# Aikku93/ulc-codec

Measured on AMD Instinct MI355X. Metric: encode+decode Msamples/s at BlockSize=2048 stereo (channel-samples through encode+decode, VBR -50, 32 blocks per stream per call), higher is better.
Workload: dtype f32; 1 GPU; vbr50 (configs[1] encode, configs[2] decode): Batch=4096 independent 44.1 kHz stereo streams/GPU x 32 blocks, BlockSize=2048, VBR -50; step = encode then decode; config=vbr50, mode=both, streams_per_gpu=4096, block_size=2048, channels=2, parallelism=batch split over 1 GPU(s), no collective on the data path

## Files before the change

ulc-codec_amd/csrc/ulcx_enc.hip:

```cpp
#include "ulcx_enc_dev.h"

static size_t ulcx_enc_xf_lds_bytes(int BS, int C) {
    if (BS > 8192) return (size_t)BS * 4;
    int ps = ulcx_xf_pad_shift(BS, C);
    size_t z = (size_t)4 * (BS + (BS >> ps)) * 4;
    size_t full = z + (size_t)BS * 2 + 32 + (C > 2 ? (size_t)BS * 2 : 0);
    return full <= ULCX_LDS_LIMIT ? full : z + (size_t)BS * 2 + 32;
}

static size_t ulcx_enc_xfa_lds_bytes(int BS, int C) {
    if (BS > 8192) return (size_t)BS * 4;
    int ps = ulcx_xf_pad_shift(BS, C);
    return (size_t)2 * (BS + (BS >> ps)) * 4 + (size_t)BS * 2 + 32;
}

#define CK(x) do { hipError_t e_ = (x); if (e_ != hipSuccess) { ulcx_set_error("%s: %s", #x, hipGetErrorString(e_)); return ULCX_ERR_HIP; } } while (0)
#define TRY(x) do { int rc_ = (x); if (rc_) return rc_; } while (0)

typedef void (*RangeKernel)(UlcxEncCtx, int, int);
typedef void (*PassKernel)(UlcxEncCtx, int);
typedef void (*CallKernel)(UlcxEncCtx);

static RangeKernel wc_energy_fn(const UlcxEncCtx &c) { return c.pcm16 ? k_wc_energy<int16_t> : k_wc_energy<float>; }
static RangeKernel wc_ef_fn(const UlcxEncCtx &c) { return c.pcm16 ? k_wc_ef<EF_NW, int16_t> : k_wc_ef<EF_NW, float>; }
// ... 25 lines not shown
    return pass == 1 ? select_fn_pass<1>(c, pair, rates) : pass == 2 ? select_fn_pass<2>(c, pair, rates) : select_fn_pass<0>(c, pair, rates);
}

static int allow_lds(const void *fn, size_t lds) {
    if (lds > 48 * 1024) CK(hipFuncSetAttribute(fn, hipFuncAttributeMaxDynamicSharedMemorySize, (int)lds));
    return ULCX_OK;
}

static void launch_wc_energy(const UlcxEncCtx &c, unsigned grid, hipStream_t st, int k0, int k1) {
    hipLaunchKernelGGL(wc_energy_fn(c), dim3(grid), dim3(WG), 0, st, c, k0, k1);
}

static void launch_wc_ef(const UlcxEncCtx &c, hipStream_t st, int k0, int k1) {
    static_assert(EF_LDS_BYTES <= 48 * 1024, "k_wc_ef: raise the dynamic LDS limit with hipFuncSetAttribute");
    hipLaunchKernelGGL(wc_ef_fn(c), dim3((c.B + EF_SPW - 1) / EF_SPW), dim3(EF_NW * 64), EF_LDS_BYTES, st, c, k0, k1);
}

static void launch_state_update(const UlcxEncCtx &c, hipStream_t st) {
    hipLaunchKernelGGL(state_update_fn(c), dim3(c.B), dim3(WG), 0, st, c);
}

const char *const ulcx_enc_stage_names[ULCX_ENC_STAGES_REPORTED] = {
    "k_wc_energy", "k_wc_forward", "k_wc_backward", "k_wc_integrate", "k_wc_decide",
    "k_xf", "k_cplx", "k_pbark", "k_mask",
    "k_select", "k_nbark", "(k_nline: gone)", "k_heapsel", "k_nsums", "k_tails", "k_encode_wave", "k_encode_units", "k_pack", "cbr_probe_passes", "k_state_update", "wc_pipeline_exposed",
};

struct StageMarks { hipEvent_t *ev; int stage; };
#define MARK(mk, s) do { if ((mk).ev) CK(hipEventRecord((mk).ev[(mk).stage++], s)); } while (0)

// ... 55 lines not shown
        hipLaunchKernelGGL(k_wc_integrate, dim3((c.B + 63) / 64), dim3(64), 0, side3, c, k0, k1);
        hipLaunchKernelGGL(k_wc_decide, dim3((c.B * kc + 63) / 64), dim3(64), 0, side3, c, k0, k1);
        CK(hipEventRecord(sy.wcDecided[w], side3));
        while (jx < nCh && cut[jx + 1] <= k1) {
            CK(hipStreamWaitEvent(st, sy.wcDecided[w], 0));
            if (mk.ev) CK(hipEventRecord(sy.xfTiming[2 * jx], st));
            if (!(ULCX_DBG(c) & 0x2000))
            transform(cut[jx], cut[jx + 1]);
            if (mk.ev) CK(hipEventRecord(sy.xfTiming[2 * jx + 1], st));
            CK(hipEventRecord(sy.xfChunkDone[jx], st));
            jx++;
        }
    }
    aux.nXf = nCh;
    MARK(mk, st);
    for (int j = 0; j < nCh; j++) {
        CK(hipStreamWaitEvent(side, sy.xfChunkDone[j], 0));
        const int kc2 = cut[j + 1] - cut[j];
        if (what == ULCX_FRONT_ENCODE) hipLaunchKernelGGL(k_cplx, dim3((c.B * kc2 + 63) / 64), dim3(64), 0, side, c, cut[j], cut[j + 1]);
        else hipLaunchKernelGGL(k_cplxa, dim3((c.B * kc2 + 63) / 64), dim3(64), 0, side, c, cut[j], cut[j + 1]);
    }
    CK(hipEventRecord(sy.cplxChunksDone, side));
    return ULCX_OK;
}

struct EncPlan {
    int NB, N, nUnits;
    bool aside;
    int probes;
    size_t barkLds;
    bool selWave, selPair;
    size_t selLds;
    int ldsEntries, fbGrid; size_t heapLds;
    WaveCaps capS, capM, capF;
    bool haveFull, haveMid;
// ... 27 lines not shown
    p.haveMid = p.capM.k < p.capF.k;
    p.nsSlots = aux.nsSlots;
    return p;
}

static void launch_noise(const UlcxEncCtx &c, const EncPlan &p, hipStream_t s2) {
    if (c.barkRing) {
        hipLaunchKernelGGL(k_bark_uniform<true>, dim3((p.NB * c.C + 63) / 64), dim3(256), p.barkLds, s2, c);
        hipLaunchKernelGGL(k_bark_levels<true>, dim3((unsigned)(((size_t)p.NB * c.C * 32 + WG - 1) / WG)), dim3(WG), 0, s2, c);
    }
    hipLaunchKernelGGL(k_nbark, dim3((p.nUnits + 63) / 64), dim3(64), 0, s2, c, c.barkRing ? 1 : 0);
}

static int launch_psy(const UlcxEncCtx &c, const EncPlan &p, UlcxEncSync &sy, hipStream_t st, StageMarks &mk, bool cplxChunked) {
    if (c.barkRing) { TRY(allow_lds((const void *)k_bark_uniform<true>, p.barkLds)); TRY(allow_lds((const void *)k_bark_uniform<false>, p.barkLds)); }
    if (p.aside) {
        CK(hipEventRecord(sy.noiseFork, st));
        CK(hipStreamWaitEvent(sy.side3, sy.noiseFork, 0));
        if (cplxChunked) CK(hipStreamWaitEvent(sy.side3, sy.cplxChunksDone, 0));
        else hipLaunchKernelGGL(k_cplx, dim3((p.NB + 63) / 64), dim3(64), 0, sy.side3, c, 0, c.K);
        CK(hipEventRecord(sy.cplxDone, sy.side3));
        MARK(mk, st);
        launch_state_update(c, sy.side3);
        CK(hipEventRecord(sy.stateDone, sy.side3));
        CK(hipStreamWaitEvent(sy.side2, sy.noiseFork, 0));
        launch_noise(c, p, sy.side2);
        CK(hipEventRecord(sy.noiseDone, sy.side2));
    } else { hipLaunchKernelGGL(k_cplx, dim3((p.NB + 63) / 64), dim3(64), 0, st, c, 0, c.K);                MARK(mk, st); }
    const bool uniP = c.barkRing != 0;
    if (uniP) {
        hipLaunchKernelGGL(k_bark_uniform<false>, dim3((p.NB + 63) / 64), dim3(256), p.barkLds, st, c);
        hipLaunchKernelGGL(k_bark_levels<false>, dim3((unsigned)(((size_t)p.NB * 32 + WG - 1) / WG)), dim3(WG), 0, st, c);
    }
    hipLaunchKernelGGL(k_pbark, dim3((p.NB * 4 + 63) / 64), dim3(64), 0, st, c, uniP ? 1 : 0);            MARK(mk, st);
    MARK(mk, st);
    if (p.aside) CK(hipStreamWaitEvent(st, sy.cplxDone, 0));
    return ULCX_OK;
}

static int launch_select_wave(const UlcxEncCtx &c, const EncPlan &p, hipStream_t st, bool rates, int pass, int fin) {
    const PassKernel fn = select_fn(c, p.selPair, rates, pass);
    TRY(allow_lds((const void *)fn, p.selLds));
    if (p.selPair) hipLaunchKernelGGL(fn, dim3(p.NB), dim3(128), p.selLds, st, c, fin);
// ... 144 lines not shown
    CK(hipGetLastError());
    return ULCX_OK;
}

int ulcx_enc_launch(const UlcxEncCtx &c, hipStream_t st, hipEvent_t *ev, const UlcxEncAux &aux) {
    return ulcx_enc_launch_ladder(&c, 1, st, ev, aux);
}

int ulcx_analyse_launch(const UlcxEncCtx &c, hipStream_t st, hipEvent_t *ev, const UlcxEncAux &aux, int useKxf) {
    const int what = !c.cplxOut ? ULCX_FRONT_WC_ONLY : useKxf ? ULCX_FRONT_ANALYSE_KXF : ULCX_FRONT_ANALYSE;
    if (what == ULCX_FRONT_ANALYSE_KXF && c.barkRing) CK(hipMemsetAsync(c.decCount, 0, sizeof(int), st));
    StageMarks mk = { ev, 0 };
    MARK(mk, st);
    TRY(launch_front(c, st, mk, aux, what));
    if (aux.wcPipe > 1) CK(hipStreamWaitEvent(st, aux.sync.cplxChunksDone, 0));
    else hipLaunchKernelGGL(k_cplxa, dim3((c.B * c.K + 63) / 64), dim3(64), 0, st, c, 0, c.K);
    MARK(mk, st);
    while (mk.ev && mk.stage < ULCX_ENC_STAGES) MARK(mk, st);
    launch_state_update(c, st);
    MARK(mk, st);
    CK(hipGetLastError());
    return ULCX_OK;
}
```

ulc-codec_amd/csrc/ulcx_enc_dev.h:

```cpp
#pragma once
#include <utility>
#include "ulcx_internal.h"

#include <type_traits>

#include "ulcx_libm.h"

#define WG 256

#define FFT_PACKED

#include "ulcx_fft.h"

__device__ __forceinline__ float fastlog(float x) {
    uint32_t b = __float_as_uint(x);
    int e = (int)(b >> 23) - 127;
    float m = __uint_as_float((127u << 23) | (b & 0x7FFFFFu));
    return -1.7417939f + (2.8212026f + (-1.4699568f + (0.44717955f - 0.056570851f * m) * m) * m) * m + 0.6931471806f * e;
}

__device__ __forceinline__ int quant_u(float v) {
    return (v >= 0.5f) ? (int)(0.5f + sqrtf(v - 0.25f)) : 0;
}

// ... 206 lines not shown
#define BK_PPR (BK_TL / 4)

#define BK_PIECES (64 * BK_PPR)

#define BK_NPC ((BK_PIECES + 191) / 192)

#ifndef BK_AHEAD

#define BK_AHEAD 4

#endif

#define BK_RS (2 * BK_TL + 4)

#define BK_TILE_FLOATS (64 * BK_RS)

__device__ __forceinline__ bool probes_over(const UlcxEncCtx &c, int finalPass) { return !finalPass && c.fbMode != 2 && *c.cbrLive <= 0; }

__device__ __forceinline__ bool skip_block(const UlcxEncCtx &c, int blk, int finalPass) {
    if (!finalPass && c.cbrDone[blk]) return true;
    if (c.fbMode == 1) return c.isFb[blk] != 0;
    return false;
}

__device__ __forceinline__ int fb_count(const UlcxEncCtx &c) {
    int n = *c.fbCount; if (n > c.fbHi) n = c.fbHi;
    n -= c.fbLo; return n > 0 ? n : 0;
}

#define ULCX_DPP_STEPS(OP) \
// ... 208 lines not shown
```

ulc-codec_amd/csrc/ulcx_enc_xf.hip:

```cpp
#include "ulcx_enc_dev.h"

__device__ __forceinline__ int first_overlap(int wc, int BS) {
    unsigned p = ulcx_pattern(wc);
    int ov = BS >> (p & 7);
    if (p & 8) ov >>= (wc & 7);
    return ov;
}

__device__ __forceinline__ float win_apply(float x, int i, int S, int aL, int ovL, int aR, int ov,
                                           const float *__restrict__ rise, const float *__restrict__ fall) {
    if (i < S) return (i < aL) ? 0.0f : (i < aL + ovL) ? x * rise[i - aL] : x;
    int n = i - S;
    return (n < aR) ? x : (n < aR + ov) ? x * fall[n - aR] : 0.0f;
}

template <typename IN, int BSC, bool AN = false>
__device__ __forceinline__ int xf_fast(const UlcxEncCtx &c, float *lds, int s, int k, int blk, int tid) {
    constexpr int BS = BSC, S = BSC, M = BSC / 2, PS = 4, Mp = FFT_PADDEDS(M, PS);
    constexpr int LGM = BSC == 4096 ? 11 : 10;
    static_assert(BSC == 2048 || BSC == 4096, "sizes with a compile-time transform");
    static_assert(WG == 256 && (M / 2) % (2 * WG) == 0, "whole fold / epilogue trips per thread");
    float2 *z = (float2 *)lds;
    float2 *twl = (float2 *)(lds + (AN ? 2 : 4) * FFT_PADDEDS(BS, PS));
    float2 *zc0 = z, *zs0 = z + Mp, *zc1 = z + (AN ? 1 : 2) * Mp, *zs1 = z + 3 * Mp;
    const float2 *pre = c.T.pre[0];
    const float *rise = c.T.winRise + S, *fall = c.T.winFall + S;
    const IN *pcmS = pcm_base<IN>(c) + (size_t)s * c.K * BS * 2;
    const IN *frameLo = pcmS + (ptrdiff_t)(k - 2) * BS * 2, *frameHi = frameLo;
    if constexpr (std::is_same<IN, float>::value) {
        const float *histS = c.hist + (size_t)s * 2 * BS * 2;
        if (k < 2) frameLo = histS + (size_t)k * BS * 2;
        if (k < 1) frameHi = histS;
// ... 28 lines not shown
                const float vl = la - lb, wl = lb + la;
                const float v1 = hsel ? vl : vr, v2 = hsel ? vr : vl;
                const float w1 = hsel ? wl : wr, w2 = hsel ? wr : wl;
                float2 *zc = q ? zc1 : zc0, *zs = q ? zs1 : zs0;
                zc[FFT_PADS(n, PS)] = cmulc(make_float2(v1, v2), P);
                if constexpr (!AN) zs[FFT_PADS(n, PS)] = cmulc(make_float2(w2, w1), P);
            }
        }
    }
    __syncthreads();
    if constexpr (AN) { if (tid < 128) fft_wave_dif_ct<M, PS>(z + __builtin_amdgcn_readfirstlane(tid >> 6) * Mp, twl, tid & 63); }
    else fft_wave_dif_ct<M, PS>(z + __builtin_amdgcn_readfirstlane(tid >> 6) * Mp, twl, tid & 63);
    __syncthreads();
    float *coefO = c.coef + (size_t)blk * (2 * BS);
    constexpr float norm = 2.0f / S;
    int nnz = 0;
    if constexpr (AN) {
#pragma unroll
        for (int e0 = 0; e0 < M / 2; e0 += 2 * WG) {
            const int kA = e0 + 2 * tid, kB = e0 + 2 * tid + 1;
            const int kk2[2] = { kA, kB };
            float re[2][2][4];
#pragma unroll
            for (int u = 0; u < 2; u++) {
                const int k1 = kk2[u], k2 = M - 1 - k1;
                const int r1 = (int)(__brev((unsigned)k1) >> (32 - LGM)), r2 = (int)(__brev((unsigned)k2) >> (32 - LGM));
                const float2 P1 = pre[k1], P2 = pre[k2];
                const fft_v2f Pv1 = { P1.x, P1.y }, Pv2 = { P2.x, P2.y };
#pragma unroll
                for (int q = 0; q < 2; q++) {
                    const float2 *zc = q ? zc1 : zc0;
// ... 2 lines not shown
                    const float mdct[4] = { yc1.x, yc2.y, yc2.x, yc1.y };
#pragma unroll
                    for (int p = 0; p < 2; p++) {
                        const int slot = p ? (1 - u) : u;
                        re[q][p][2 * slot] = mdct[2*p] * norm; re[q][p][2 * slot + 1] = mdct[2*p+1] * norm;
                    }
                }
            }
            const int j1 = kA, j2 = M - 1 - kB;
#pragma unroll
            for (int q = 0; q < 2; q++) {
                stnt((float4 *)(coefO + q * BS + 2 * j1), make_float4(re[q][0][0], re[q][0][1], re[q][0][2], re[q][0][3]));
                stnt((float4 *)(coefO + q * BS + 2 * j2), make_float4(re[q][1][0], re[q][1][1], re[q][1][2], re[q][1][3]));
            }
        }
        return 0;
    }
#pragma unroll
    for (int e0 = 0; e0 < M / 2; e0 += 2 * WG) {
        const int kA = e0 + 2 * tid, kB = e0 + 2 * tid + 1;
        const int kk2[2] = { kA, kB };
        float re[2][2][4];
        float ns[2][2][2];
        float am[2][2] = { { 0.0f, 0.0f }, { 0.0f, 0.0f } };
#pragma unroll
        for (int u = 0; u < 2; u++) {
            const int k1 = kk2[u], k2 = M - 1 - k1;
            const int r1 = (int)(__brev((unsigned)k1) >> (32 - LGM)), r2 = (int)(__brev((unsigned)k2) >> (32 - LGM));
            const float2 P1 = pre[k1], P2 = pre[k2];
            const fft_v2f Pv1 = { P1.x, P1.y }, Pv2 = { P2.x, P2.y };
#pragma unroll
            for (int q = 0; q < 2; q++) {
                const float2 *zc = q ? zc1 : zc0, *zs = q ? zs1 : zs0;
                auto cm = [](float2 d, fft_v2f w) { const fft_v2f dv = { d.x, d.y }; const fft_v2f r = fft_cmulc_post_pk(dv, w); return make_float2(r.x, r.y); };
                const float2 yc1 = cm(zc[FFT_PADS(r1, PS)], Pv1), yc2 = cm(zc[FFT_PADS(r2, PS)], Pv2);
                const float2 ys1 = cm(zs[FFT_PADS(r1, PS)], Pv1), ys2 = cm(zs[FFT_PADS(r2, PS)], Pv2);
                const float mdct[4] = { yc1.x, yc2.y, yc2.x, yc1.y };
                const float mdst[4] = { ys1.x, ys2.y, ys2.x, ys1.y };
#pragma unroll
                for (int p = 0; p < 2; p++) {
                    const float re0 = mdct[2*p] * norm,   im0 = mdst[2*p] * norm;
                    const float re1 = mdct[2*p+1] * norm, im1 = mdst[2*p+1] * norm;
                    const float re0s = re0 * re0, im0s = im0 * im0, re1s = re1 * re1, im1s = im1 * im1;
                    const float a0 = re0s + im0s, a1 = re1s + im1s;
                    nnz += (fabsf(re0) < 0.5f * ULCX_COEF_EPS) ? 0 : 1;
                    nnz += (fabsf(re1) < 0.5f * ULCX_COEF_EPS) ? 0 : 1;
                    const int slot = p ? (1 - u) : u;
                    re[q][p][2 * slot] = re0; re[q][p][2 * slot + 1] = re1;
                    ns[q][p][slot] = a0 + a1;
                    am[p][slot] += a0; am[p][slot] += a1;
                }
            }
        }
        const int j1 = kA, j2 = M - 1 - kB;
#pragma unroll
        for (int q = 0; q < 2; q++) {
            stnt((float4 *)(coefO + q * BS + 2 * j1), make_float4(re[q][0][0], re[q][0][1], re[q][0][2], re[q][0][3]));
            stnt((float4 *)(coefO + q * BS + 2 * j2), make_float4(re[q][1][0], re[q][1][1], re[q][1][2], re[q][1][3]));
            stnt((float2 *)(c.nsum + tile_idx(BS / 2, blk * 2 + q, j1)), make_float2(ns[q][0][0], ns[q][0][1]));
            stnt((float2 *)(c.nsum + tile_idx(BS / 2, blk * 2 + q, j2)), make_float2(ns[q][1][0], ns[q][1][1]));
        }
        *(float2 *)(c.amp2 + tile_idx(BS / 2, blk, j1)) = make_float2(am[0][0], am[0][1]);
        *(float2 *)(c.amp2 + tile_idx(BS / 2, blk, j2)) = make_float2(am[1][0], am[1][1]);
    }
    return nnz;
}

template <typename IN>
__device__ __forceinline__ bool xf_is_fast(const UlcxEncCtx &c, int s, int k) {
#ifdef XF_NO_FAST
    return false;
#endif
    const int BS = c.BS;
    const int *wrow = c.wcArr + (size_t)s * (c.maxK + 2) + k;
    const int wcPrev = wrow[0], wc = wrow[1], wcNext = wrow[2];
    if (!(k >= 2 || std::is_same<IN, float>::value) || (ulcx_pattern(wc) >> 4) != 0) return false;
    unsigned pp = ulcx_pattern(wcPrev);
    int lastS = BS;
    do { lastS = BS >> (pp & 7); } while (pp >>= 4);
    int ovFirst = first_overlap(wc, BS);
    if (ovFirst > lastS) ovFirst = lastS;
    return ovFirst == BS && first_overlap(wcNext, BS) >= BS;
}

template <bool ST, typename IN, bool AN = false>
__device__ __forceinline__ void xf_block(const UlcxEncCtx &c, float *lds, int s, int k, const int tid) {
    const int BS = c.BS, C = ST ? 2 : c.C;
    const int blk = s * c.K + k;
    const int ps = ulcx_xf_pad_shift(BS, C);
    float2 *z    = (float2 *)lds;
    constexpr int NA = AN ? 2 : 4;
    float2 *twl  = (float2 *)(lds + NA * FFT_PADDEDS(BS, ps));
    int    &s_nnz = *(int *)(lds + NA * FFT_PADDEDS(BS, ps) + BS / 2);
    const bool ampLds = !AN && (C > 2);
    const bool twInLds = !(ampLds && (size_t)16 * (BS + (BS >> ps)) + (size_t)BS * 4 + 32 > ULCX_LDS_LIMIT);
    float  *amp2 = twInLds ? lds + 4 * FFT_PADDEDS(BS, ps) + BS / 2 + 4 : lds + 4 * FFT_PADDEDS(BS, ps);
    if (!AN && tid == 0) s_nnz = 0;
    if (ampLds) for (int i = tid; i < BS / 2; i += WG) amp2[i] = 0.0f;

    const int *wrow = c.wcArr + (size_t)s * (c.maxK + 2) + k;
    int wcPrev = wrow[0], wc = wrow[1], wcNext = wrow[2];
    if (!AN && c.barkRing && tid == 0 && (ulcx_pattern(wc) & ~8u) != 0) c.decList[atomicAdd(c.decCount, 1)] = blk;
    int nextOv = first_overlap(wcNext, BS);
    int ovFirst;
    {
        unsigned pp = ulcx_pattern(wcPrev);
        int lastS = BS;
        do { lastS = BS >> (pp & 7); } while (pp >>= 4);
        ovFirst = first_overlap(wc, BS);
        if (ovFirst > lastS) ovFirst = lastS;
    }
    size_t cb = (size_t)C * BS;
    float *coefO = c.coef + (size_t)blk * cb;
    int nnz = 0;
    __syncthreads();

#ifdef XF_NO_FAST
    const bool fastBlk = false;
#else
    const bool fastBlk = ST && (BS == 2048 || BS == 4096) && (k >= 2 || std::is_same<IN, float>::value) && (ulcx_pattern(wc) >> 4) == 0
                         && ovFirst == BS && nextOv >= BS;
#endif
    if (fastBlk) nnz = (BS == 2048) ? xf_fast<IN, 2048, AN>(c, lds, s, k, blk, tid) : xf_fast<IN, 4096, AN>(c, lds, s, k, blk, tid);
    else
    for (int ch0 = 0; ch0 < C; ch0 += 2) {
        const int nch = ST ? 2 : ((ch0 + 1 < C) ? 2 : 1);
        unsigned pat = ulcx_pattern(wc);
        int off = 0, ovL = ovFirst;
        do {
            int S = BS >> (pat & 7);
            int d = pat & 7;
            pat >>= 4;
            int ov;
            if (pat) { ov = BS >> (pat & 7); if (pat & 8) ov >>= (wc & 7); }
            else ov = nextOv;
            if (ov > S) ov = S;
            const int M = S >> 1;
            int t0 = (k - 1) * BS - BS / 2 + off - S / 2;
// ... 109 lines not shown
                        for (int p = 0; p < 2; p++) {
                            const int j = p ? k2 : k1;
                            stnt((float2 *)(coefO + (size_t)ch * BS + off + 2 * j), make_float2(mdctA[2*p] * norm, mdctA[2*p+1] * norm));
                        }
                        continue;
                    }
                    float2 ys1 = cm(zs[FFT_PADS(r1, ps)], Pv1), ys2 = cm(zs[FFT_PADS(r2, ps)], Pv2);
                    float mdct[4] = { yc1.x, yc2.y, yc2.x, yc1.y };
                    float mdst[4] = { ys1.x, ys2.y, ys2.x, ys1.y };
#pragma unroll
                    for (int p = 0; p < 2; p++) {
                        float re0 = mdct[2*p] * norm,   im0 = mdst[2*p] * norm;
                        float re1 = mdct[2*p+1] * norm, im1 = mdst[2*p+1] * norm;
                        float re0s = re0 * re0, im0s = im0 * im0, re1s = re1 * re1, im1s = im1 * im1;
                        float a0 = re0s + im0s, a1 = re1s + im1s;
                        nnz += (fabsf(re0) < 0.5f * ULCX_COEF_EPS) ? 0 : 1;
                        nnz += (fabsf(re1) < 0.5f * ULCX_COEF_EPS) ? 0 : 1;
                        int j = p ? k2 : k1;
                        size_t gi = (size_t)ch * BS + off + 2 * j;
                        stnt((float2 *)(coefO + gi), make_float2(re0, re1));
                        stnt(c.nsum + tile_idx(BS / 2, blk * C + ch, off / 2 + j), a0 + a1);
                        if (p) { am2 += a0; am2 += a1; } else { am1 += a0; am1 += a1; }
                    }
                }
                if (AN) continue;
                if (ampLds) { amp2[off / 2 + k1] = am1; amp2[off / 2 + k2] = am2; }
                else { c.amp2[tile_idx(BS / 2, blk, off / 2 + k1)] = am1; c.amp2[tile_idx(BS / 2, blk, off / 2 + k2)] = am2; }
            }
            __syncthreads();
            off += S; ovL = ov;
        } while (pat);
    }
    if (AN) return;
    for (int o = 32; o > 0; o >>= 1) nnz += __shfl_down(nnz, o);
    if ((tid & 63) == 0) atomicAdd(&s_nnz, nnz);
    if (ampLds) for (int i = tid; i < BS / 2; i += WG) c.amp2[tile_idx(BS / 2, blk, i)] = amp2[i];
    __syncthreads();
    if (tid == 0) c.nnz[blk] = s_nnz;
}

#ifndef ULCX_XF_ANALYSIS_UNIT
template <bool ST, typename IN>
__global__ __launch_bounds__(WG, 4) void k_xf(UlcxEncCtx c, int k0, int k1) {
    extern __shared__ float lds[];
    const int kc = k1 - k0;
    const int NBk = c.B * kc;
    const int per = (NBk + 7) / 8;
    const int vb = (int)(blockIdx.x % 8) * per + (int)(blockIdx.x / 8);
    if (vb >= NBk) return;
    xf_block<ST, IN>(c, lds, vb / kc, k0 + vb % kc, threadIdx.x);
}
#else
template <bool ST, typename IN>
// ... 8 lines not shown
}
#endif

template <typename IN, bool AN>
__device__ __forceinline__ void xf_big_block(const UlcxEncCtx &c, int k0, int k1) {
    extern __shared__ float lds[];
    const int BS = c.BS, C = c.C;
    const int kc = k1 - k0;
    const int NBk = c.B * kc;
    const int vb = blockIdx.x;
    if (vb >= NBk) return;
    const int s = vb / kc, k = k0 + vb % kc;
    const int blk = s * c.K + k;
    const int tid = threadIdx.x;
    float2 *z = (float2 *)lds;
    __shared__ int s_nnz;
    if (tid == 0) s_nnz = 0;
    const int *wrow = c.wcArr + (size_t)s * (c.maxK + 2) + k;
    const int wcPrev = wrow[0], wc = wrow[1], wcNext = wrow[2];
    if (!AN && c.barkRing && threadIdx.x == 0 && (ulcx_pattern(wc) & ~8u) != 0) c.decList[atomicAdd(c.decCount, 1)] = blk;
    const int nextOv = first_overlap(wcNext, BS);
    int ovFirst;
    {
        unsigned pp = ulcx_pattern(wcPrev);
        int lastS = BS;
        do { lastS = BS >> (pp & 7); } while (pp >>= 4);
        ovFirst = first_overlap(wc, BS);
        if (ovFirst > lastS) ovFirst = lastS;
    }
    const size_t cb = (size_t)C * BS;
    float *coefO = c.coef + (size_t)blk * cb;
    int nnz = 0;
    __syncthreads();
    for (int ch = 0; ch < C; ch++) {
        unsigned pat = ulcx_pattern(wc);
        int off = 0, ovL = ovFirst;
        do {
            const int S = BS >> (pat & 7);
            const int d = pat & 7;
            pat >>= 4;
            int ov;
            if (pat) { ov = BS >> (pat & 7); if (pat & 8) ov >>= (wc & 7); }
            else ov = nextOv;
            if (ov > S) ov = S;
            const int M = S >> 1;
            const int t0 = (k - 1) * BS - BS / 2 + off - S / 2;
            const int aL = (S - ovL) >> 1, aR = (S - ov) >> 1;
            const float *rise = c.T.winRise + ovL, *fall = c.T.winFall + ov;
// ... 21 lines not shown
                }
                __syncthreads();
                fftn_dif(z, 1, M, c.T.tw[d], tid);
                for (int kk = tid; kk < M / 2; kk += WG) {
                    const int kA = kk, kB = M - 1 - kk;
                    const int r1 = (int)(__brev((unsigned)kA) >> (32 - bits));
                    const int r2 = (int)(__brev((unsigned)kB) >> (32 - bits));
                    const float2 y1 = cmulc_post(z[r1], pre[kA]), y2 = cmulc_post(z[r2], pre[kB]);
#pragma unroll
                    for (int p = 0; p < 2; p++) {
                        const int j = p ? kB : kA;
                        const size_t gi = (size_t)ch * BS + off + 2 * j;
                        if (kind == 0) {
                            const float m0 = p ? y2.x : y1.x, m1 = p ? y1.y : y2.y;
                            const float re0 = m0 * norm, re1 = m1 * norm;
                            nnz += (fabsf(re0) < 0.5f * ULCX_COEF_EPS) ? 0 : 1;
                            nnz += (fabsf(re1) < 0.5f * ULCX_COEF_EPS) ? 0 : 1;
                            *(float2 *)(coefO + gi) = make_float2(re0, re1);
                        } else {
                            const float m0 = p ? y2.x : y1.x, m1 = p ? y1.y : y2.y;
                            const float im0 = m0 * norm, im1 = m1 * norm;
                            const float2 re = *(const float2 *)(coefO + gi);
                            const float re0s = re.x * re.x, im0s = im0 * im0, re1s = re.y * re.y, im1s = im1 * im1;
                            const float a0 = re0s + im0s, a1 = re1s + im1s;
                            c.nsum[tile_idx(BS / 2, blk * C + ch, off / 2 + j)] = a0 + a1;
                            float *ap = c.amp2 + tile_idx(BS / 2, blk, off / 2 + j);
                            float am = (ch == 0) ? 0.0f : *ap;
                            am += a0; am += a1;
                            *ap = am;
                        }
                    }
                }
                __syncthreads();
            }
            off += S; ovL = ov;
        } while (pat);
    }
    if (AN) return;
    for (int o = 32; o > 0; o >>= 1) nnz += __shfl_down(nnz, o);
    if ((tid & 63) == 0) atomicAdd(&s_nnz, nnz);
    __syncthreads();
    if (tid == 0) c.nnz[blk] = s_nnz;
}

#ifndef ULCX_XF_ANALYSIS_UNIT
template <typename IN>
__global__ __launch_bounds__(WG) void k_xf_big(UlcxEncCtx c, int k0, int k1) {
    xf_big_block<IN, false>(c, k0, k1);
}
#else
template <typename IN>
__global__ __launch_bounds__(WG) void k_xfa_big(UlcxEncCtx c, int k0, int k1) {
    xf_big_block<IN, true>(c, k0, k1);
}
#endif

#ifndef ULCX_XF_ANALYSIS_UNIT
__global__ __launch_bounds__(64) void k_cplx(UlcxEncCtx c, int k0, int k1) {
    const int gidc = blockIdx.x * 64 + threadIdx.x, kcc = k1 - k0;
    if (gidc >= c.B * kcc) return;
    const int blk = (gidc / kcc) * c.K + k0 + gidc % kcc;
    int n = c.C * c.BS;
    const float4 *p = (const float4 *)(c.coef + (size_t)blk * n);
    float cx = 0.0f, cw = 0.0f;
    int tiny = 0;
    auto sums = [&](auto tinyT) {
        constexpr bool TINY = decltype(tinyT)::value;
        for (int i = 0; i < n / 4; i += 4) {
            float4 q[4];
#pragma unroll
            for (int u = 0; u < 4; u++) q[u] = p[i + u];
#pragma unroll
            for (int u = 0; u < 4; u++) {
                float4 v = q[u];
                cx += v.x * v.x; cw += fabsf(v.x);
                cx += v.y * v.y; cw += fabsf(v.y);
                cx += v.z * v.z; cw += fabsf(v.z);
                cx += v.w * v.w; cw += fabsf(v.w);
                if (TINY) {
                    tiny += (fabsf(v.x) >= 0.5f * ULCX_COEF_EPS && fabsf(v.x) < 0x1.0p-29f) ? 1 : 0;
                    tiny += (fabsf(v.y) >= 0.5f * ULCX_COEF_EPS && fabsf(v.y) < 0x1.0p-29f) ? 1 : 0;
                    tiny += (fabsf(v.z) >= 0.5f * ULCX_COEF_EPS && fabsf(v.z) < 0x1.0p-29f) ? 1 : 0;
                    tiny += (fabsf(v.w) >= 0.5f * ULCX_COEF_EPS && fabsf(v.w) < 0x1.0p-29f) ? 1 : 0;
                }
            }
        }
    };
    int mode = c.mode;
    float p0 = c.p0, p1 = c.p1, vbrTarget = c.vbrTarget;
    if (c.rates) {
        const float2 r = c.rates[blk / c.K];
        if (r.x < 0.0f) {
            mode = ULCX_MODE_VBR; p0 = -r.x;
            vbrTarget = 0x1.E4EFB7p3f * ulcx_logf(100.0f / p0);
        } else { mode = (r.y > 0.0f) ? ULCX_MODE_ABR : ULCX_MODE_CBR; p0 = r.x; p1 = r.y; }
        if (__ballot(mode != ULCX_MODE_VBR)) sums(std::true_type{}); else sums(std::false_type{});
    } else if (c.mode == ULCX_MODE_VBR) sums(std::false_type{}); else sums(std::true_type{});
    if (cx != 0.0f) {
        cx = ulcx_logf((cw * cw) / cx) / c.cplxScale;
        if (cx < 0.0f) cx = 0.0f;
        if (cx > 1.0f) cx = 1.0f;
    }
    c.cplx[blk] = cx;
    int maxCoef = c.nnz[blk];
    if (mode == ULCX_MODE_VBR) {
        int nT = maxCoef;
        if (vbrTarget > 0.0f) {
            float ft = (c.C * c.BS) * cx / vbrTarget;
            if (ft < maxCoef) nT = (int)ft;
        }
        c.nout[blk] = nT;
        if (c.rates) {
            c.cbrLo[blk] = 0; c.cbrHi[blk] = maxCoef;
            c.cbrDone[blk] = ULCX_DONE_VBR;
            c.cbrBudget[blk] = 0;
            c.selWin[blk] = make_uint4(0u, 0u, (uint32_t)(c.C * c.BS), 0u);
            for (int u = 0; u < c.C * 4; u++) c.tailSum[((size_t)blk * c.C * 4 + u) * 8 + 6] = 0.0f;
        }
    } else {
        float kbps = p0;
        if (mode == ULCX_MODE_ABR) kbps = p0 * cx / p1;
        int budget = (int)((c.BS * kbps) * 1000.0f / c.rateHz);
        int lo = 0, hi = maxCoef;
        int done = (0 < maxCoef) ? 0 : 1;
        int nOut = (0 < maxCoef) ? (int)((unsigned)(0 + maxCoef) / 2u) : 0;
        while (!done && 4 * (nOut - tiny + 1) > budget) {
            hi = nOut - 1;
            if (!(lo < hi - 1)) { done = 1; nOut = lo; }
            else nOut = (int)((unsigned)(lo + hi) / 2u);
        }
        c.cbrLo[blk] = lo; c.cbrHi[blk] = hi;
        c.cbrDone[blk] = done;
        c.selWin[blk] = make_uint4(0u, 0u, (uint32_t)(c.C * c.BS), 0u);
        for (int u = 0; u < c.C * 4; u++) c.tailSum[((size_t)blk * c.C * 4 + u) * 8 + 6] = 0.0f;
        {
            const unsigned long long open = __ballot(!done);
            if (open && (int)__builtin_amdgcn_mbcnt_hi((uint32_t)(open >> 32), __builtin_amdgcn_mbcnt_lo((uint32_t)open, 0u)) == 0 && !done)
                atomicAdd(c.cbrLive, (int)__popcll(open));
        }
        c.nout[blk] = nOut;
        c.cbrBudget[blk] = budget;
    }
    c.isFb[blk] = 0;
    if (c.useWave) c.slow[blk] = 0;
    if (blk == 0) { *c.fbCount = 0; if (c.useWave) { c.slow[c.B * c.K] = 0; c.slow[c.B * c.K + 1] = 0; } }
    int s = blk / c.K, k = blk % c.K;
    if (c.wcOut)   c.wcOut[blk]   = c.wcArr[(size_t)s * (c.maxK + 2) + k + 1];
    if (c.cplxOut) c.cplxOut[blk] = cx;
}

#else
__global__ __launch_bounds__(64) void k_cplxa(UlcxEncCtx c, int k0, int k1) {
    const int gidc = blockIdx.x * 64 + threadIdx.x, kcc = k1 - k0;
    if (gidc >= c.B * kcc) return;
    const int s = gidc / kcc, k = k0 + gidc % kcc;
    const int blk = s * c.K + k;
    if (c.wcOut) c.wcOut[blk] = c.wcArr[(size_t)s * (c.maxK + 2) + k + 1];
    if (!c.cplxOut) return;
    const int n = c.C * c.BS;
    const float4 *p = (const float4 *)(c.coef + (size_t)blk * n);
    float cx = 0.0f, cw = 0.0f;
    for (int i = 0; i < n / 4; i += 4) {
        float4 q[4];
#pragma unroll
        for (int u = 0; u < 4; u++) q[u] = p[i + u];
#pragma unroll
        for (int u = 0; u < 4; u++) {
            float4 v = q[u];
            cx += v.x * v.x; cw += fabsf(v.x);
            cx += v.y * v.y; cw += fabsf(v.y);
            cx += v.z * v.z; cw += fabsf(v.z);
            cx += v.w * v.w; cw += fabsf(v.w);
        }
    }
    if (cx != 0.0f) {
        cx = ulcx_logf((cw * cw) / cx) / c.cplxScale;
        if (cx < 0.0f) cx = 0.0f;
        if (cx > 1.0f) cx = 1.0f;
    }
    c.cplxOut[blk] = cx;
}
#endif

#ifndef ULCX_XF_ANALYSIS_UNIT
template <typename IN>
__global__ __launch_bounds__(WG) void k_state_update(UlcxEncCtx c) {
    int s = blockIdx.x, tid = threadIdx.x;
    int n = 2 * c.BS * c.C;
    float *h = c.hist + (size_t)s * n;
    int newF = c.K * c.BS * c.C;
    const IN *p = pcm_base<IN>(c) + (size_t)s * newF;
    if (c.K >= 2) {
        for (int i = tid; i < n; i += WG) h[i] = ld1(p + newF - n + i);
    } else {
        int half = n / 2;
        for (int i = tid; i < half; i += WG) { h[i] = h[half + i]; h[half + i] = ld1(p + i); }
// ... 28 lines not shown
```

Baseline: 56210 Msamples/s.

## Stage k_cplx coefficient rows through LDS with producer waves; move nnz count into cplx

The complexity kernel now runs 256-thread workgroups. Three producer waves prefetch coefficient tiles from 64 rows into double-buffered LDS, which turns the old one-row-per-thread strided float4 reads into coalesced loads, and one consumer wave reduces the tiles. The nonzero-coefficient count moves out of the transform kernels and into this pass, which removes a shuffle reduction, an LDS atomic and a barrier per transform block. In exchange the cplx kernel gains a barrier per tile, extra LDS, and three waves that only load.

```diff
diff --git a/ulc-codec_amd/csrc/ulcx_enc.hip b/ulc-codec_amd/csrc/ulcx_enc.hip
--- a/ulc-codec_amd/csrc/ulcx_enc.hip
+++ b/ulc-codec_amd/csrc/ulcx_enc.hip
@@ -63,6 +63,11 @@
 static void launch_wc_ef(const UlcxEncCtx &c, hipStream_t st, int k0, int k1) {
     static_assert(EF_LDS_BYTES <= 48 * 1024, "k_wc_ef: raise the dynamic LDS limit with hipFuncSetAttribute");
     hipLaunchKernelGGL(wc_ef_fn(c), dim3((c.B + EF_SPW - 1) / EF_SPW), dim3(EF_NW * 64), EF_LDS_BYTES, st, c, k0, k1);
+}
+
+static RangeKernel cplx_fn(bool analysis) { return analysis ? k_cplxa : k_cplx; }
+static void launch_cplx(RangeKernel fn, const UlcxEncCtx &c, hipStream_t st, int k0, int k1) {
+    hipLaunchKernelGGL(fn, dim3((c.B * (k1 - k0) + 63) / 64), dim3(256), CX_LDS_BYTES, st, c, k0, k1);
 }
 
 static void launch_state_update(const UlcxEncCtx &c, hipStream_t st) {
@@ -148,11 +153,11 @@
     }
     aux.nXf = nCh;
     MARK(mk, st);
+    const RangeKernel cplx = cplx_fn(what != ULCX_FRONT_ENCODE);
+    TRY(allow_lds((const void *)cplx, CX_LDS_BYTES));
     for (int j = 0; j < nCh; j++) {
         CK(hipStreamWaitEvent(side, sy.xfChunkDone[j], 0));
-        const int kc2 = cut[j + 1] - cut[j];
-        if (what == ULCX_FRONT_ENCODE) hipLaunchKernelGGL(k_cplx, dim3((c.B * kc2 + 63) / 64), dim3(64), 0, side, c, cut[j], cut[j + 1]);
-        else hipLaunchKernelGGL(k_cplxa, dim3((c.B * kc2 + 63) / 64), dim3(64), 0, side, c, cut[j], cut[j + 1]);
+        launch_cplx(cplx, c, side, cut[j], cut[j + 1]);
     }
     CK(hipEventRecord(sy.cplxChunksDone, side));
     return ULCX_OK;
@@ -210,11 +215,12 @@
 
 static int launch_psy(const UlcxEncCtx &c, const EncPlan &p, UlcxEncSync &sy, hipStream_t st, StageMarks &mk, bool cplxChunked) {
     if (c.barkRing) { TRY(allow_lds((const void *)k_bark_uniform<true>, p.barkLds)); TRY(allow_lds((const void *)k_bark_uniform<false>, p.barkLds)); }
+    if (!cplxChunked) TRY(allow_lds((const void *)cplx_fn(false), CX_LDS_BYTES));
     if (p.aside) {
         CK(hipEventRecord(sy.noiseFork, st));
         CK(hipStreamWaitEvent(sy.side3, sy.noiseFork, 0));
         if (cplxChunked) CK(hipStreamWaitEvent(sy.side3, sy.cplxChunksDone, 0));
-        else hipLaunchKernelGGL(k_cplx, dim3((p.NB + 63) / 64), dim3(64), 0, sy.side3, c, 0, c.K);
+        else launch_cplx(cplx_fn(false), c, sy.side3, 0, c.K);
         CK(hipEventRecord(sy.cplxDone, sy.side3));
         MARK(mk, st);
         launch_state_update(c, sy.side3);
@@ -222,7 +228,7 @@
         CK(hipStreamWaitEvent(sy.side2, sy.noiseFork, 0));
         launch_noise(c, p, sy.side2);
         CK(hipEventRecord(sy.noiseDone, sy.side2));
-    } else { hipLaunchKernelGGL(k_cplx, dim3((p.NB + 63) / 64), dim3(64), 0, st, c, 0, c.K);                MARK(mk, st); }
+    } else { launch_cplx(cplx_fn(false), c, st, 0, c.K);                                                 MARK(mk, st); }
     const bool uniP = c.barkRing != 0;
     if (uniP) {
         hipLaunchKernelGGL(k_bark_uniform<false>, dim3((p.NB + 63) / 64), dim3(256), p.barkLds, st, c);
@@ -397,7 +403,7 @@
     MARK(mk, st);
     TRY(launch_front(c, st, mk, aux, what));
     if (aux.wcPipe > 1) CK(hipStreamWaitEvent(st, aux.sync.cplxChunksDone, 0));
-    else hipLaunchKernelGGL(k_cplxa, dim3((c.B * c.K + 63) / 64), dim3(64), 0, st, c, 0, c.K);
+    else { TRY(allow_lds((const void *)cplx_fn(true), CX_LDS_BYTES)); launch_cplx(cplx_fn(true), c, st, 0, c.K); }
     MARK(mk, st);
     while (mk.ev && mk.stage < ULCX_ENC_STAGES) MARK(mk, st);
     launch_state_update(c, st);
diff --git a/ulc-codec_amd/csrc/ulcx_enc_dev.h b/ulc-codec_amd/csrc/ulcx_enc_dev.h
--- a/ulc-codec_amd/csrc/ulcx_enc_dev.h
+++ b/ulc-codec_amd/csrc/ulcx_enc_dev.h
@@ -244,6 +244,20 @@
 #define BK_RS (2 * BK_TL + 4)
 
 #define BK_TILE_FLOATS (64 * BK_RS)
+
+#ifndef CX_TL
+#define CX_TL 128
+#endif
+#ifndef CX_AHEAD
+#define CX_AHEAD 2
+#endif
+#define CX_PPR (CX_TL / 4)
+#define CX_PIECES (64 * CX_PPR)
+#define CX_NPC ((CX_PIECES + 191) / 192)
+#define CX_RS (CX_TL + 4)
+#define CX_TILE_FLOATS (64 * CX_RS)
+#define CX_LDS_BYTES ((size_t)2 * CX_TILE_FLOATS * 4)
+static_assert(256 % CX_TL == 0 && CX_TL % 64 == 0, "CX_TL: 64, 128 or 256");
 
 __device__ __forceinline__ bool probes_over(const UlcxEncCtx &c, int finalPass) { return !finalPass && c.fbMode != 2 && *c.cbrLive <= 0; }
 
diff --git a/ulc-codec_amd/csrc/ulcx_enc_xf.hip b/ulc-codec_amd/csrc/ulcx_enc_xf.hip
--- a/ulc-codec_amd/csrc/ulcx_enc_xf.hip
+++ b/ulc-codec_amd/csrc/ulcx_enc_xf.hip
@@ -15,7 +15,7 @@
 }
 
 template <typename IN, int BSC, bool AN = false>
-__device__ __forceinline__ int xf_fast(const UlcxEncCtx &c, float *lds, int s, int k, int blk, int tid) {
+__device__ __forceinline__ void xf_fast(const UlcxEncCtx &c, float *lds, int s, int k, int blk, int tid) {
     constexpr int BS = BSC, S = BSC, M = BSC / 2, PS = 4, Mp = FFT_PADDEDS(M, PS);
     constexpr int LGM = BSC == 4096 ? 11 : 10;
     static_assert(BSC == 2048 || BSC == 4096, "sizes with a compile-time transform");
@@ -74,7 +74,6 @@
     __syncthreads();
     float *coefO = c.coef + (size_t)blk * (2 * BS);
     constexpr float norm = 2.0f / S;
-    int nnz = 0;
     if constexpr (AN) {
 #pragma unroll
         for (int e0 = 0; e0 < M / 2; e0 += 2 * WG) {
@@ -107,7 +106,7 @@
                 stnt((float4 *)(coefO + q * BS + 2 * j2), make_float4(re[q][1][0], re[q][1][1], re[q][1][2], re[q][1][3]));
             }
         }
-        return 0;
+        return;
     }
 #pragma unroll
     for (int e0 = 0; e0 < M / 2; e0 += 2 * WG) {
@@ -136,8 +135,6 @@
                     const float re1 = mdct[2*p+1] * norm, im1 = mdst[2*p+1] * norm;
                     const float re0s = re0 * re0, im0s = im0 * im0, re1s = re1 * re1, im1s = im1 * im1;
                     const float a0 = re0s + im0s, a1 = re1s + im1s;
-                    nnz += (fabsf(re0) < 0.5f * ULCX_COEF_EPS) ? 0 : 1;
-                    nnz += (fabsf(re1) < 0.5f * ULCX_COEF_EPS) ? 0 : 1;
                     const int slot = p ? (1 - u) : u;
                     re[q][p][2 * slot] = re0; re[q][p][2 * slot + 1] = re1;
                     ns[q][p][slot] = a0 + a1;
@@ -156,7 +153,6 @@
         *(float2 *)(c.amp2 + tile_idx(BS / 2, blk, j1)) = make_float2(am[0][0], am[0][1]);
         *(float2 *)(c.amp2 + tile_idx(BS / 2, blk, j2)) = make_float2(am[1][0], am[1][1]);
     }
-    return nnz;
 }
 
 template <typename IN>
@@ -184,11 +180,9 @@
     float2 *z    = (float2 *)lds;
     constexpr int NA = AN ? 2 : 4;
     float2 *twl  = (float2 *)(lds + NA * FFT_PADDEDS(BS, ps));
-    int    &s_nnz = *(int *)(lds + NA * FFT_PADDEDS(BS, ps) + BS / 2);
     const bool ampLds = !AN && (C > 2);
     const bool twInLds = !(ampLds && (size_t)16 * (BS + (BS >> ps)) + (size_t)BS * 4 + 32 > ULCX_LDS_LIMIT);
     float  *amp2 = twInLds ? lds + 4 * FFT_PADDEDS(BS, ps) + BS / 2 + 4 : lds + 4 * FFT_PADDEDS(BS, ps);
-    if (!AN && tid == 0) s_nnz = 0;
     if (ampLds) for (int i = tid; i < BS / 2; i += WG) amp2[i] = 0.0f;
 
     const int *wrow = c.wcArr + (size_t)s * (c.maxK + 2) + k;
@@ -205,7 +199,6 @@
     }
     size_t cb = (size_t)C * BS;
     float *coefO = c.coef + (size_t)blk * cb;
-    int nnz = 0;
     __syncthreads();
 
 #ifdef XF_NO_FAST
@@ -214,7 +207,7 @@
     const bool fastBlk = ST && (BS == 2048 || BS == 4096) && (k >= 2 || std::is_same<IN, float>::value) && (ulcx_pattern(wc) >> 4) == 0
                          && ovFirst == BS && nextOv >= BS;
 #endif
-    if (fastBlk) nnz = (BS == 2048) ? xf_fast<IN, 2048, AN>(c, lds, s, k, blk, tid) : xf_fast<IN, 4096, AN>(c, lds, s, k, blk, tid);
+    if (fastBlk) { if (BS == 2048) xf_fast<IN, 2048, AN>(c, lds, s, k, blk, tid); else xf_fast<IN, 4096, AN>(c, lds, s, k, blk, tid); }
     else
     for (int ch0 = 0; ch0 < C; ch0 += 2) {
         const int nch = ST ? 2 : ((ch0 + 1 < C) ? 2 : 1);
@@ -354,8 +347,6 @@
                         float re1 = mdct[2*p+1] * norm, im1 = mdst[2*p+1] * norm;
                         float re0s = re0 * re0, im0s = im0 * im0, re1s = re1 * re1, im1s = im1 * im1;
                         float a0 = re0s + im0s, a1 = re1s + im1s;
-                        nnz += (fabsf(re0) < 0.5f * ULCX_COEF_EPS) ? 0 : 1;
-                        nnz += (fabsf(re1) < 0.5f * ULCX_COEF_EPS) ? 0 : 1;
                         int j = p ? k2 : k1;
                         size_t gi = (size_t)ch * BS + off + 2 * j;
                         stnt((float2 *)(coefO + gi), make_float2(re0, re1));
@@ -372,11 +363,7 @@
         } while (pat);
     }
     if (AN) return;
-    for (int o = 32; o > 0; o >>= 1) nnz += __shfl_down(nnz, o);
-    if ((tid & 63) == 0) atomicAdd(&s_nnz, nnz);
     if (ampLds) for (int i = tid; i < BS / 2; i += WG) c.amp2[tile_idx(BS / 2, blk, i)] = amp2[i];
-    __syncthreads();
-    if (tid == 0) c.nnz[blk] = s_nnz;
 }
 
 #ifndef ULCX_XF_ANALYSIS_UNIT
@@ -415,8 +402,6 @@
     const int blk = s * c.K + k;
     const int tid = threadIdx.x;
     float2 *z = (float2 *)lds;
-    __shared__ int s_nnz;
-    if (tid == 0) s_nnz = 0;
     const int *wrow = c.wcArr + (size_t)s * (c.maxK + 2) + k;
     const int wcPrev = wrow[0], wc = wrow[1], wcNext = wrow[2];
     if (!AN && c.barkRing && threadIdx.x == 0 && (ulcx_pattern(wc) & ~8u) != 0) c.decList[atomicAdd(c.decCount, 1)] = blk;
@@ -431,8 +416,6 @@
     }
     const size_t cb = (size_t)C * BS;
     float *coefO = c.coef + (size_t)blk * cb;
-    int nnz = 0;
-    __syncthreads();
     for (int ch = 0; ch < C; ch++) {
         unsigned pat = ulcx_pattern(wc);
         int off = 0, ovL = ovFirst;
@@ -484,8 +467,6 @@
                         if (kind == 0) {
                             const float m0 = p ? y2.x : y1.x, m1 = p ? y1.y : y2.y;
                             const float re0 = m0 * norm, re1 = m1 * norm;
-                            nnz += (fabsf(re0) < 0.5f * ULCX_COEF_EPS) ? 0 : 1;
-                            nnz += (fabsf(re1) < 0.5f * ULCX_COEF_EPS) ? 0 : 1;
                             *(float2 *)(coefO + gi) = make_float2(re0, re1);
                         } else {
                             const float m0 = p ? y2.x : y1.x, m1 = p ? y1.y : y2.y;
@@ -506,11 +487,6 @@
             off += S; ovL = ov;
         } while (pat);
     }
-    if (AN) return;
-    for (int o = 32; o > 0; o >>= 1) nnz += __shfl_down(nnz, o);
-    if ((tid & 63) == 0) atomicAdd(&s_nnz, nnz);
-    __syncthreads();
-    if (tid == 0) c.nnz[blk] = s_nnz;
 }
 
 #ifndef ULCX_XF_ANALYSIS_UNIT
@@ -525,131 +501,174 @@
 }
 #endif
 
-#ifndef ULCX_XF_ANALYSIS_UNIT
-__global__ __launch_bounds__(64) void k_cplx(UlcxEncCtx c, int k0, int k1) {
-    const int gidc = blockIdx.x * 64 + threadIdx.x, kcc = k1 - k0;
-    if (gidc >= c.B * kcc) return;
+typedef float cx_v4 __attribute__((ext_vector_type(4)));
+template <bool AN>
+__device__ __forceinline__ void cplx_rows(const UlcxEncCtx &c, const int k0, const int k1) {
+    extern __shared__ float cx_lds[];
+    __shared__ int s_blk[64];
+    const int tid = threadIdx.x, lane = tid & 63, wv = __builtin_amdgcn_readfirstlane(tid >> 6);
+    const int kcc = k1 - k0, nRows = c.B * kcc;
+    const bool mine = (int)blockIdx.x * 64 + lane < nRows;
+    const int gidc = min((int)blockIdx.x * 64 + lane, nRows - 1);
     const int blk = (gidc / kcc) * c.K + k0 + gidc % kcc;
-    int n = c.C * c.BS;
-    const float4 *p = (const float4 *)(c.coef + (size_t)blk * n);
+    const int n = c.C * c.BS, nTiles = n / CX_TL;
+    if constexpr (AN) {
+        if (wv == 0 && mine && c.wcOut) c.wcOut[blk] = c.wcArr[(size_t)(blk / c.K) * (c.maxK + 2) + (blk % c.K) + 1];
+        if (!c.cplxOut) return;
+    }
+    if (wv == 0) s_blk[lane] = blk;
+    __syncthreads();
+    if (wv > 0) {
+        const int p0 = (wv - 1) * 64 + lane;
+        constexpr int AH = CX_AHEAD;
+        cx_v4 nx[AH][CX_NPC];
+        auto fetch = [&](cx_v4 (&r)[CX_NPC], int t) {
+#pragma unroll
+            for (int i = 0; i < CX_NPC; i++) {
+                const int pc = p0 + 192 * i;
+                if (wv - 1 + 3 * i < CX_PIECES / 64) r[i] = *(const cx_v4 *)(c.coef + (size_t)s_blk[pc / CX_PPR] * n + t * CX_TL + (pc % CX_PPR) * 4);
+            }
+        };
+        auto put = [&](const cx_v4 (&r)[CX_NPC], int t) {
+            float *tile = cx_lds + (t & 1) * CX_TILE_FLOATS;
+#pragma unroll
+            for (int i = 0; i < CX_NPC; i++) {
+                const int pc = p0 + 192 * i;
+                if (wv - 1 + 3 * i < CX_PIECES / 64) *(cx_v4 *)(tile + (pc / CX_PPR) * CX_RS + (pc % CX_PPR) * 4) = r[i];
+            }
+        };
+#pragma unroll
+        for (int a = 0; a < AH; a++) if (a < nTiles) fetch(nx[a], a);
+        put(nx[0], 0);
+        if (AH < nTiles) fetch(nx[0], AH);
+        __syncthreads();
+        for (int t0 = 0; t0 < nTiles; t0 += AH) {
+#pragma unroll
+            for (int a = 0; a < AH; a++) {
+                const int t = t0 + a;
+                if (t < nTiles) {
+                    if (t + 1 < nTiles) { put(nx[(a + 1) % AH], t + 1); if (t + 1 + AH < nTiles) fetch(nx[(a + 1) % AH], t + 1 + AH); }
+                    __syncthreads();
+                }
+            }
+        }
+        return;
+    }
     float cx = 0.0f, cw = 0.0f;
-    int tiny = 0;
+    int tiny = 0, nnz = 0;
     auto sums = [&](auto tinyT) {
         constexpr bool TINY = decltype(tinyT)::value;
-        for (int i = 0; i < n / 4; i += 4) {
-            float4 q[4];
-#pragma unroll
-            for (int u = 0; u < 4; u++) q[u] = p[i + u];
-#pragma unroll
-            for (int u = 0; u < 4; u++) {
-                float4 v = q[u];
-                cx += v.x * v.x; cw += fabsf(v.x);
-                cx += v.y * v.y; cw += fabsf(v.y);
-                cx += v.z * v.z; cw += fabsf(v.z);
-                cx += v.w * v.w; cw += fabsf(v.w);
-                if (TINY) {
-                    tiny += (fabsf(v.x) >= 0.5f * ULCX_COEF_EPS && fabsf(v.x) < 0x1.0p-29f) ? 1 : 0;
-                    tiny += (fabsf(v.y) >= 0.5f * ULCX_COEF_EPS && fabsf(v.y) < 0x1.0p-29f) ? 1 : 0;
-                    tiny += (fabsf(v.z) >= 0.5f * ULCX_COEF_EPS && fabsf(v.z) < 0x1.0p-29f) ? 1 : 0;
-                    tiny += (fabsf(v.w) >= 0.5f * ULCX_COEF_EPS && fabsf(v.w) < 0x1.0p-29f) ? 1 : 0;
+        __syncthreads();
+        for (int t = 0; t < nTiles; t++) {
+            const float4 *p = (const float4 *)(cx_lds + (t & 1) * CX_TILE_FLOATS + lane * CX_RS);
+            for (int i = 0; i < CX_TL / 4; i += 4) {
+                float4 q[4];
+#pragma unroll
+                for (int u = 0; u < 4; u++) q[u] = p[i + u];
+#pragma unroll
+                for (int u = 0; u < 4; u++) {
+                    float4 v = q[u];
+                    cx += v.x * v.x; cw += fabsf(v.x);
+                    cx += v.y * v.y; cw += fabsf(v.y);
+                    cx += v.z * v.z; cw += fabsf(v.z);
+                    cx += v.w * v.w; cw += fabsf(v.w);
+                    if constexpr (!AN) {
+                        nnz += (fabsf(v.x) < 0.5f * ULCX_COEF_EPS) ? 0 : 1;
+                        nnz += (fabsf(v.y) < 0.5f * ULCX_COEF_EPS) ? 0 : 1;
+                        nnz += (fabsf(v.z) < 0.5f * ULCX_COEF_EPS) ? 0 : 1;
+                        nnz += (fabsf(v.w) < 0.5f * ULCX_COEF_EPS) ? 0 : 1;
+                    }
+                    if (TINY) {
+                        tiny += (fabsf(v.x) >= 0.5f * ULCX_COEF_EPS && fabsf(v.x) < 0x1.0p-29f) ? 1 : 0;
+                        tiny += (fabsf(v.y) >= 0.5f * ULCX_COEF_EPS && fabsf(v.y) < 0x1.0p-29f) ? 1 : 0;
+                        tiny += (fabsf(v.z) >= 0.5f * ULCX_COEF_EPS && fabsf(v.z) < 0x1.0p-29f) ? 1 : 0;
+                        tiny += (fabsf(v.w) >= 0.5f * ULCX_COEF_EPS && fabsf(v.w) < 0x1.0p-29f) ? 1 : 0;
+                    }
                 }
             }
+            __syncthreads();
         }
     };
-    int mode = c.mode;
-    float p0 = c.p0, p1 = c.p1, vbrTarget = c.vbrTarget;
-    if (c.rates) {
-        const float2 r = c.rates[blk / c.K];
-        if (r.x < 0.0f) {
-            mode = ULCX_MODE_VBR; p0 = -r.x;
-            vbrTarget = 0x1.E4EFB7p3f * ulcx_logf(100.0f / p0);
-        } else { mode = (r.y > 0.0f) ? ULCX_MODE_ABR : ULCX_MODE_CBR; p0 = r.x; p1 = r.y; }
-        if (__ballot(mode != ULCX_MODE_VBR)) sums(std::true_type{}); else sums(std::false_type{});
-    } else if (c.mode == ULCX_MODE_VBR) sums(std::false_type{}); else sums(std::true_type{});
-    if (cx != 0.0f) {
-        cx = ulcx_logf((cw * cw) / cx) / c.cplxScale;
-        if (cx < 0.0f) cx = 0.0f;
-        if (cx > 1.0f) cx = 1.0f;
-    }
-    c.cplx[blk] = cx;
-    int maxCoef = c.nnz[blk];
-    if (mode == ULCX_MODE_VBR) {
-        int nT = maxCoef;
-        if (vbrTarget > 0.0f) {
-            float ft = (c.C * c.BS) * cx / vbrTarget;
-            if (ft < maxCoef) nT = (int)ft;
-        }
-        c.nout[blk] = nT;
+    if constexpr (AN) {
+        sums(std::false_type{});
+        if (!mine) return;
+        if (cx != 0.0f) {
+            cx = ulcx_logf((cw * cw) / cx) / c.cplxScale;
+            if (cx < 0.0f) cx = 0.0f;
+            if (cx > 1.0f) cx = 1.0f;
+        }
+        c.cplxOut[blk] = cx;
+    } else {
+        int mode = c.mode;
+        float p0 = c.p0, p1 = c.p1, vbrTarget = c.vbrTarget;
         if (c.rates) {
-            c.cbrLo[blk] = 0; c.cbrHi[blk] = maxCoef;
-            c.cbrDone[blk] = ULCX_DONE_VBR;
-            c.cbrBudget[blk] = 0;
+            const float2 r = c.rates[blk / c.K];
+            if (r.x < 0.0f) {
+                mode = ULCX_MODE_VBR; p0 = -r.x;
+                vbrTarget = 0x1.E4EFB7p3f * ulcx_logf(100.0f / p0);
+            } else { mode = (r.y > 0.0f) ? ULCX_MODE_ABR : ULCX_MODE_CBR; p0 = r.x; p1 = r.y; }
+            if (__ballot(mode != ULCX_MODE_VBR)) sums(std::true_type{}); else sums(std::false_type{});
+        } else if (c.mode == ULCX_MODE_VBR) sums(std::false_type{}); else sums(std::true_type{});
+        if (!mine) return;
+        if (cx != 0.0f) {
+            cx = ulcx_logf((cw * cw) / cx) / c.cplxScale;
+            if (cx < 0.0f) cx = 0.0f;
+            if (cx > 1.0f) cx = 1.0f;
+        }
+        c.cplx[blk] = cx;
+        c.nnz[blk] = nnz;
+        int maxCoef = nnz;
+        if (mode == ULCX_MODE_VBR) {
+            int nT = maxCoef;
+            if (vbrTarget > 0.0f) {
+                float ft = (c.C * c.BS) * cx / vbrTarget;
+                if (ft < maxCoef) nT = (int)ft;
+            }
+            c.nout[blk] = nT;
+            if (c.rates) {
+                c.cbrLo[blk] = 0; c.cbrHi[blk] = maxCoef;
+                c.cbrDone[blk] = ULCX_DONE_VBR;
+                c.cbrBudget[blk] = 0;
+                c.selWin[blk] = make_uint4(0u, 0u, (uint32_t)(c.C * c.BS), 0u);
+                for (int u = 0; u < c.C * 4; u++) c.tailSum[((size_t)blk * c.C * 4 + u) * 8 + 6] = 0.0f;
+            }
+        } else {
+            float kbps = p0;
+            if (mode == ULCX_MODE_ABR) kbps = p0 * cx / p1;
+            int budget = (int)((c.BS * kbps) * 1000.0f / c.rateHz);
+            int lo = 0, hi = maxCoef;
+            int done = (0 < maxCoef) ? 0 : 1;
+            int nOut = (0 < maxCoef) ? (int)((unsigned)(0 + maxCoef) / 2u) : 0;
+            while (!done && 4 * (nOut - tiny + 1) > budget) {
+                hi = nOut - 1;
+                if (!(lo < hi - 1)) { done = 1; nOut = lo; }
+                else nOut = (int)((unsigned)(lo + hi) / 2u);
+            }
+            c.cbrLo[blk] = lo; c.cbrHi[blk] = hi;
+            c.cbrDone[blk] = done;
             c.selWin[blk] = make_uint4(0u, 0u, (uint32_t)(c.C * c.BS), 0u);
             for (int u = 0; u < c.C * 4; u++) c.tailSum[((size_t)blk * c.C * 4 + u) * 8 + 6] = 0.0f;
-        }
-    } else {
-        float kbps = p0;
-        if (mode == ULCX_MODE_ABR) kbps = p0 * cx / p1;
-        int budget = (int)((c.BS * kbps) * 1000.0f / c.rateHz);
-        int lo = 0, hi = maxCoef;
-        int done = (0 < maxCoef) ? 0 : 1;
-        int nOut = (0 < maxCoef) ? (int)((unsigned)(0 + maxCoef) / 2u) : 0;
-        while (!done && 4 * (nOut - tiny + 1) > budget) {
-            hi = nOut - 1;
-            if (!(lo < hi - 1)) { done = 1; nOut = lo; }
-            else nOut = (int)((unsigned)(lo + hi) / 2u);
-        }
-        c.cbrLo[blk] = lo; c.cbrHi[blk] = hi;
-        c.cbrDone[blk] = done;
-        c.selWin[blk] = make_uint4(0u, 0u, (uint32_t)(c.C * c.BS), 0u);
-        for (int u = 0; u < c.C * 4; u++) c.tailSum[((size_t)blk * c.C * 4 + u) * 8 + 6] = 0.0f;
-        {
-            const unsigned long long open = __ballot(!done);
-            if (open && (int)__builtin_amdgcn_mbcnt_hi((uint32_t)(open >> 32), __builtin_amdgcn_mbcnt_lo((uint32_t)open, 0u)) == 0 && !done)
-                atomicAdd(c.cbrLive, (int)__popcll(open));
-        }
-        c.nout[blk] = nOut;
-        c.cbrBudget[blk] = budget;
-    }
-    c.isFb[blk] = 0;
-    if (c.useWave) c.slow[blk] = 0;
-    if (blk == 0) { *c.fbCount = 0; if (c.useWave) { c.slow[c.B * c.K] = 0; c.slow[c.B * c.K + 1] = 0; } }
-    int s = blk / c.K, k = blk % c.K;
-    if (c.wcOut)   c.wcOut[blk]   = c.wcArr[(size_t)s * (c.maxK + 2) + k + 1];
-    if (c.cplxOut) c.cplxOut[blk] = cx;
-}
-
+            {
+                const unsigned long long open = __ballot(!done);
+                if (open && (int)__builtin_amdgcn_mbcnt_hi((uint32_t)(open >> 32), __builtin_amdgcn_mbcnt_lo((uint32_t)open, 0u)) == 0 && !done)
+                    atomicAdd(c.cbrLive, (int)__popcll(open));
+            }
+            c.nout[blk] = nOut;
+            c.cbrBudget[blk] = budget;
+        }
+        c.isFb[blk] = 0;
+        if (c.useWave) c.slow[blk] = 0;
+        if (blk == 0) { *c.fbCount = 0; if (c.useWave) { c.slow[c.B * c.K] = 0; c.slow[c.B * c.K + 1] = 0; } }
+        int s = blk / c.K, k = blk % c.K;
+        if (c.wcOut)   c.wcOut[blk]   = c.wcArr[(size_t)s * (c.maxK + 2) + k + 1];
+        if (c.cplxOut) c.cplxOut[blk] = cx;
+    }
+}
+
+#ifndef ULCX_XF_ANALYSIS_UNIT
+__global__ __launch_bounds__(256) void k_cplx(UlcxEncCtx c, int k0, int k1) { cplx_rows<false>(c, k0, k1); }
 #else
-__global__ __launch_bounds__(64) void k_cplxa(UlcxEncCtx c, int k0, int k1) {
-    const int gidc = blockIdx.x * 64 + threadIdx.x, kcc = k1 - k0;
-    if (gidc >= c.B * kcc) return;
-    const int s = gidc / kcc, k = k0 + gidc % kcc;
-    const int blk = s * c.K + k;
-    if (c.wcOut) c.wcOut[blk] = c.wcArr[(size_t)s * (c.maxK + 2) + k + 1];
-    if (!c.cplxOut) return;
-    const int n = c.C * c.BS;
-    const float4 *p = (const float4 *)(c.coef + (size_t)blk * n);
-    float cx = 0.0f, cw = 0.0f;
-    for (int i = 0; i < n / 4; i += 4) {
-        float4 q[4];
-#pragma unroll
-        for (int u = 0; u < 4; u++) q[u] = p[i + u];
-#pragma unroll
-        for (int u = 0; u < 4; u++) {
-            float4 v = q[u];
-            cx += v.x * v.x; cw += fabsf(v.x);
-            cx += v.y * v.y; cw += fabsf(v.y);
-            cx += v.z * v.z; cw += fabsf(v.z);
-            cx += v.w * v.w; cw += fabsf(v.w);
-        }
-    }
-    if (cx != 0.0f) {
-        cx = ulcx_logf((cw * cw) / cx) / c.cplxScale;
-        if (cx < 0.0f) cx = 0.0f;
-        if (cx > 1.0f) cx = 1.0f;
-    }
-    c.cplxOut[blk] = cx;
-}
+__global__ __launch_bounds__(256) void k_cplxa(UlcxEncCtx c, int k0, int k1) { cplx_rows<true>(c, k0, k1); }
 #endif
 
 #ifndef ULCX_XF_ANALYSIS_UNIT
```

Result: slower. 54290 Msamples/s (-3.4%).
